# kubeflow/Code-Intelligence

Hardware: NVIDIA H100
Metric: issues/sec to 2400-d @ seq_len 512 batch 256 (higher is better)
Workload: dtype bf16

## Files before the change

code_intelligence_b200/csrc/api.cu:

```cuda
#include <algorithm>
#include <cmath>
#include <cstdarg>
#include <cstdio>
#include <cstdlib>
#include <cstring>
#include <mutex>
#include <string>
#include <vector>

#include <cuda_fp16.h>

#include "../../include/issue_emb_b200.h"
#include "kernels.h"

namespace {

thread_local std::string g_last_error;

int fail(int code, const char* fmt, ...) {
  char buf[512];
  va_list ap;
  va_start(ap, fmt);
  vsnprintf(buf, sizeof(buf), fmt, ap);
  va_end(ap);
// ... 375 lines not shown
    }
    if ((rc = mark(h, 1, s)) != IE_OK) return rc;
    int cur = 0;
    const __nv_bfloat16* layer_in = h->x0.as<__nv_bfloat16>();
    const __nv_bfloat16* prev_ring = nullptr;
    long long layer_in_ld = ring_mul * h->e_pad;
    for (int l = 0; l < c.n_layers; ++l) {
      const bool last = (l == c.n_layers - 1);
      Layer& L = h->layers[l];
      const bool from_table = proj && l == 0;
      const bool fused = persistent && last && l > 0 && h->segs == 1 && h->fuse_last && L.w_cat.p != nullptr;
      __nv_bfloat16* ybuf = h->y[cur].as<__nv_bfloat16>();
      __nv_bfloat16* carry = h->hcarry.as<__nv_bfloat16>() + static_cast<size_t>(l) * carry_layer;
      float* cstate = h->c.as<float>() + static_cast<size_t>(l) * h->max_batch * mop;
      CUtensorMap tm_h, tm_w;
      CK(ie::make_tmap_bf16_2d(&tm_h, ybuf, static_cast<uint64_t>(ring_mul) * L.kh_pad, static_cast<uint64_t>(crow + b_pad),
                               h->y_ld, 64, 128));
      if (fused)
        CK(ie::make_tmap_bf16_2d(&tm_w, L.w_cat.p, static_cast<uint64_t>(L.kin_pad + L.kh_pad), 4ull * L.out_pad,
                                 static_cast<uint64_t>(L.kin_pad + L.kh_pad), 64, 256));
      else
        CK(ie::make_tmap_bf16_2d(&tm_w, L.w_hh.p, static_cast<uint64_t>(ring_mul) * L.kh_pad, 4ull * L.out_pad,
                                 static_cast<uint64_t>(ring_mul) * L.kh_pad, 64, 256));
      CUtensorMap tm_h64 = tm_h;
      CUtensorMap tm_x = tm_h;
      if (fused)
        CK(ie::make_tmap_bf16_2d(&tm_x, prev_ring, static_cast<uint64_t>(L.kin_pad), static_cast<uint64_t>(crow + b_pad),
                                 h->y_ld, 64, 128));
      if (h->use_mc)
        CK(ie::make_tmap_bf16_2d(&tm_h64, ybuf, static_cast<uint64_t>(ring_mul) * L.kh_pad,
                                 static_cast<uint64_t>(crow + b_pad), h->y_ld, 64, 64));
      CK(cudaMemcpyAsync(ybuf, carry, slot_bytes, cudaMemcpyDeviceToDevice, s));
      if (!from_table && !fused) {
        ie::GemmArgs g{};
        fill_gemm(h, L, g);
        g.a = layer_in;
        g.lda = layer_in_ld;
        g.d = h->gx.p;
        g.m_pad = static_cast<int>(crow);
        g.m_store = static_cast<int>(crow);
        g.diag = h->diag.as<long long>() + 8 * l + 4;
        CK(ie::launch_gemm_bf16(g, s));
        h->launches++;
      }
      if ((rc = mark(h, 2 + 2 * l, s)) != IE_OK) return rc;

      if (persistent) CK(cudaMemsetAsync(h->step_done.p, 0, static_cast<size_t>(Tc) * ng * sizeof(unsigned), s));
      ie::LstmLayerArgs q{};
      q.tm_h = tm_h; q.tm_w = tm_w; q.tm_h64 = tm_h64; q.mc = h->use_mc; q.mc_ctas = h->mc_ctas;
      q.tm_x = tm_x; q.pre_nkb = fused ? L.kin_pad / 64 : 0; q.bias = L.bias.as<float>();
      q.gx = from_table ? h->proj.p : h->gx.p;
      q.tok = from_table ? h->tok.as<int>() : nullptr;
      q.c = cstate; q.y = ybuf;
      q.raw = (l == raw_layer && raw_out != nullptr) ? h->raw.as<float>() : nullptr;
      q.pool_sum = (last && pooled) ? h->pool_sum.as<float>() : nullptr;
      q.pool_max = h->pool_max.as<float>(); q.pool_last = h->pool_last.as<float>();
      q.lengths = h->lengths.as<int>();
      q.step_done = h->step_done.as<unsigned>();
      q.abort_flag = h->err.as<unsigned>() + 1; q.spin_limit = h->spin_limit;
      q.T = Tc; q.t0 = static_cast<int>(t0); q.T_total = T; q.ng = ng;
      q.u = L.u; q.n_cta = L.n_cta; q.out_pad = L.out_pad; q.kh_pad = L.kh_pad;
      q.ldy = h->y_ld; q.raw_ld = L.out_pad;
      q.gate_mode = h->gate_mode; q.gx_bf16 = h->gx_bf16; q.segs = h->segs;
      q.num_sms = h->num_sms; q.check_only = 0; q.cooperative = h->cooperative; q.fault = h->fault;
      q.diag = h->diag.as<long long>() + 8 * l;
// ... 844 lines not shown
```

code_intelligence_b200/csrc/gemm.cu:

```cuda
#include "gemm_kernel.cuh"

namespace ie {


cudaError_t launch_gemm_bf16(const GemmArgs& g, cudaStream_t stream) {
  if (g.m_pad % kBlockM || g.k_pad % kBlockK || g.bn % 16 || g.bn < 16 || g.bn > 256 || g.n_pad % g.bn ||
      g.n_store % 16 || g.ldd % 2)
    return cudaErrorInvalidValue;
  CUtensorMap tmA, tmB;
  const int segs = g.segs == 3 ? 3 : 1;
  const uint64_t k_inner = static_cast<uint64_t>(segs == 3 ? 2 : 1) * g.k_pad;
  const long long spin_limit = g.spin_limit > 0 ? g.spin_limit : kSpinLimitDefault;
  cudaError_t e = make_tmap_bf16_2d(&tmA, g.a, k_inner, g.m_pad, g.lda, kBlockK, kBlockM);
  if (e != cudaSuccess) return e;
  e = make_tmap_bf16_2d(&tmB, g.b, k_inner, g.n_pad, g.ldb, kBlockK, kBlockN);
  if (e != cudaSuccess) return e;

  const size_t smem = 1024 + static_cast<size_t>(kGemmStages) * kGemmStageBytes + 2 * kGemmStages * 8 + 32;
  const int num_m_blocks = g.m_pad / kBlockM;
  const int num_n_blocks = (g.n_pad + kBlockN - 1) / kBlockN;
  const int num_k_blocks = g.k_pad / kBlockK;
  const int num_tiles = num_m_blocks * num_n_blocks;
  const int sms = g.num_sms > 0 ? g.num_sms : 132;
  const int grid = num_tiles < sms ? num_tiles : sms;
  const int panel = 16;

#define IE_LAUNCH(OUT, ACT, FRAG)                                                                                  \
  do {                                                                                                             \
    auto kfn = gemm_bf16_kernel<OUT, ACT, FRAG>;                                                                       \
    e = cudaFuncSetAttribute(kfn, cudaFuncAttributeMaxDynamicSharedMemorySize, static_cast<int>(smem));            \
// ... 30 lines not shown
```

code_intelligence_b200/csrc/kernels.h:

```cpp
#pragma once
#include <cuda.h>
#include <cuda_bf16.h>
#include <cuda_runtime.h>
#include <stddef.h>
#include <stdint.h>

namespace ie {

cudaError_t make_tmap_bf16_2d(CUtensorMap* out, const void* base, uint64_t inner, uint64_t rows, uint64_t ld,
                              uint32_t box_inner, uint32_t box_rows);

__host__ __device__ inline int frag_index(int c, int elem_bytes) {
  const int q = (c & 7) >> 1;
  const int ix = 4 * (c >> 4) + 2 * ((c >> 3) & 1) + (c & 1);
  const int per_chunk = 16 / elem_bytes;
  return (ix / per_chunk * 4 + q) * per_chunk + ix % per_chunk;
}

struct GemmArgs {
  const __nv_bfloat16* a;
  const __nv_bfloat16* b;
  void* d;
  const float* bias;
  int m_pad, n_pad, k_pad;
  long long lda, ldb, ldd;
// ... 4 lines not shown
  int num_sms;
  int segs;
  unsigned* abort_flag;
  long long spin_limit;
  long long* diag;
  int frag;
};
cudaError_t launch_gemm_bf16(const GemmArgs& g, cudaStream_t stream);

constexpr int kMaxBatches = 12;
struct LstmLayerArgs {
  CUtensorMap tm_h;
  CUtensorMap tm_w;
  CUtensorMap tm_h64;
  CUtensorMap tm_x;
  int pre_nkb;
  const float* bias;
  int mc;
  int mc_ctas;
  const void* gx;
  const int* tok;
  float* c;
  __nv_bfloat16* y;
  float* raw;
  float* pool_sum;
  float* pool_max;
  float* pool_last;
  const int* lengths;
  unsigned* step_done;
  unsigned* abort_flag;
// ... 61 lines not shown
```

code_intelligence_b200/csrc/knn.cu:

```cuda
#include <algorithm>

#include "gemm_kernel.cuh"

namespace ie {

namespace {

__device__ __forceinline__ uint32_t order_key(float s) {
  const uint32_t b = __float_as_uint(s);
  return (b & 0x80000000u) ? ~b : (b | 0x80000000u);
}
__device__ __forceinline__ float key_score(uint32_t k) {
  return __uint_as_float((k & 0x80000000u) ? (k & 0x7fffffffu) : ~k);
}

__device__ __noinline__ float knn_compact(uint2* buf, int count, int kp, int lane) {
  __syncwarp();
  uint32_t t = 0;
  for (int bit = 31; bit >= 0; --bit) {
    const uint32_t c = t | (1u << bit);
    int m = 0;
    for (int i = lane; i < count; i += 32) m += buf[i].x >= c;
    if (static_cast<int>(__reduce_add_sync(~0u, static_cast<unsigned>(m))) >= kp) t = c;
  }
// ... 375 lines not shown
}

void knn_plan(int nq, long long n, int kp, int num_sms, int* S, int* nbs) {
  const int m_blocks = (nq + 127) / 128;
  const long long n_blocks = (n + 255) / 256;
  long long s = std::max(1, num_sms / m_blocks);
  s = std::min<long long>(s, n_blocks);
  s = std::min<long long>(s, kKnnMergeMax / kp);
  *nbs = static_cast<int>((n_blocks + s - 1) / s);
  *S = static_cast<int>((n_blocks + *nbs - 1) / *nbs);
}

cudaError_t launch_knn_stage1(const KnnStage1Args& a, cudaStream_t stream) {
  if (a.m_pad % 128 || a.k_pad % 64 || a.nq > a.m_pad) return cudaErrorInvalidValue;
  CUtensorMap tmA, tmB;
  cudaError_t e = make_tmap_bf16_2d(&tmA, a.qs, 2ull * a.k_pad, a.m_pad, 2ull * a.k_pad, kBlockK, kBlockM);
  if (e != cudaSuccess) return e;
  e = make_tmap_bf16_2d(&tmB, a.xs, 2ull * a.k_pad, static_cast<uint64_t>(a.n), 2ull * a.k_pad, kBlockK, kBlockN);
  if (e != cudaSuccess) return e;
  KnnEpi epi{};
  epi.cand = a.cand;
  epi.cnt = a.cnt;
  epi.col = a.col;
  epi.rowt = a.rowt;
  epi.nq = a.nq;
  epi.n = static_cast<int>(a.n);
  epi.S = a.S;
  epi.nbs = a.nbs;
  epi.kp = a.kp;
  epi.cosine = a.cosine;
  epi.m_blocks = a.m_pad / kBlockM;
  epi.items = epi.m_blocks * a.S;
  const int num_n_blocks = static_cast<int>((a.n + kBlockN - 1) / kBlockN);
// ... 25 lines not shown
```

code_intelligence_b200/csrc/lstm_common.cuh:

```cuda
#pragma once
#include <cuda_bf16.h>
#include <cuda_fp16.h>

#include "ptx.cuh"

namespace ie {

constexpr int kGatesFast = 2;
constexpr int kGatesExp = 1;
constexpr int kGatesIeee = 0;

__device__ __forceinline__ float sigmoid_ieee(float x) { return 1.0f / (1.0f + expf(-x)); }
__device__ __forceinline__ float tanh_ieee(float x) {
  const float ax = fabsf(x);
  float t;
  if (ax < 0.55f) {
    const float e = expm1f(2.0f * ax);
    t = e / (e + 2.0f);
  } else {
    t = 1.0f - 2.0f / (expf(2.0f * ax) + 1.0f);
  }
  return copysignf(t, x);
}

// ... 5 lines not shown
  } else if (gate_mode == kGatesExp) {
    cnew = sigmoid_acc(zf) * cprev + sigmoid_acc(zi) * tanh_acc(zg);
    hn = sigmoid_acc(zo) * tanh_acc(cnew);
  } else {
    cnew = sigmoid_ieee(zf) * cprev + sigmoid_ieee(zi) * tanh_ieee(zg);
    hn = sigmoid_ieee(zo) * tanh_ieee(cnew);
  }
}

__device__ __forceinline__ void red_add_v4_f32(float* p, float4 v) {
  asm volatile("red.relaxed.gpu.global.add.v4.f32 [%0], {%1, %2, %3, %4};" ::"l"(p), "f"(v.x), "f"(v.y), "f"(v.z),
               "f"(v.w)
               : "memory");
}
__device__ __forceinline__ void pool_accumulate4(float* pool_sum, float* pool_max, float* pool_last, long long po,
                                                 float4 hn, int tg, int len) {
  if (tg >= len) return;
  float4* mp = reinterpret_cast<float4*>(pool_max + po);
  if (tg == 0) {
    __stcg(reinterpret_cast<float4*>(pool_sum + po), hn);
    __stcg(mp, hn);
  } else {
    red_add_v4_f32(pool_sum + po, hn);
    const float4 m = __ldcg(mp);
    __stcg(mp, make_float4(fmaxf(m.x, hn.x), fmaxf(m.y, hn.y), fmaxf(m.z, hn.z), fmaxf(m.w, hn.w)));
  }
  if (tg == len - 1) __stcg(reinterpret_cast<float4*>(pool_last + po), hn);
}

__device__ __forceinline__ uint32_t enc_max(float x) {
  const uint32_t b = __float_as_uint(x);
  return (b & 0x80000000u) ? ~b : (b | 0x80000000u);
}
__host__ __device__ __forceinline__ float dec_max(uint32_t e) {
  const uint32_t b = (e & 0x80000000u) ? (e & 0x7FFFFFFFu) : ~e;
#ifdef __CUDA_ARCH__
  return __uint_as_float(b);
#else
  float f;
// ... 15 lines not shown
```

code_intelligence_b200/csrc/lstm_layer.cu:

```cuda
#include <cmath>

#include <cuda_fp16.h>

#include "kernels.h"
#include "lstm_common.cuh"
#include "ptx.cuh"

namespace ie {

namespace {

constexpr int kLThreads = 384;
constexpr int kLStages = 4;
constexpr int kLTileN = 256;
constexpr int kLRows = 128;
constexpr uint32_t kHBytes = kLRows * 64 * 2;
constexpr uint32_t kWBytes = kLTileN * 64 * 2;
constexpr uint32_t kStageBytes = kHBytes + kWBytes;

__device__ __forceinline__ void st_release_cta(uint32_t* p, uint32_t v) {
  asm volatile("st.release.cta.shared::cta.u32 [%0], %1;" ::"r"(smem_u32(p)), "r"(v) : "memory");
}
__device__ __forceinline__ uint32_t ld_acquire_cta(const uint32_t* p) {
  uint32_t v;
  asm volatile("ld.acquire.cta.shared::cta.u32 %0, [%1];" : "=r"(v) : "r"(smem_u32(p)) : "memory");
  return v;
}
__device__ __forceinline__ void wait_seq_ge(const uint32_t* p, uint32_t target, const Abort& ab) {
  if (ld_acquire_cta(p) >= target) return;
  if (aborted(ab)) return;
  const long long t0 = clock64();
  uint32_t spins = 0;
  while (ld_acquire_cta(p) < target) {
// ... 13 lines not shown
  float* pool_max;
  float* pool_last;
  const int* lengths;
  unsigned* step_done;
  unsigned* abort_flag;
  long long spin_limit;
  long long ldy, raw_ld;
  long long* trace;
  long long* diag;
  int T, t_begin, t0, T_total, ng, tiles, out_pad, nkb, segs, kh_pad, gate_mode, trace_items, fault;
  int pre_nkb;
};

template <bool TOK, bool GXBF, bool POOL, bool MC, bool FUSE>
__device__ __forceinline__ void lstm_layer_body(const CUtensorMap& tm_h, const CUtensorMap& tm_w,
                                                const CUtensorMap& tm_h64, const CUtensorMap& tm_x, const KArgs& a) {
  extern __shared__ uint8_t smem_raw[];
  const uint32_t rawaddr = smem_u32(smem_raw);
  uint8_t* smem = smem_raw + ((1024u - (rawaddr & 1023u)) & 1023u);

  uint8_t* ring = smem;
  uint64_t* full = reinterpret_cast<uint64_t*>(ring + kLStages * kStageBytes);
  uint64_t* empty = full + kLStages;
  uint32_t* cready = reinterpret_cast<uint32_t*>(empty + kLStages);
  uint32_t* abort_s = cready + 1;
  const Abort ab{abort_s, a.abort_flag, a.spin_limit};

  const int warp = threadIdx.x >> 5;
  const int lane = threadIdx.x & 31;
  long long* const trace = a.trace;
#define IE_TRACE(slot, kk) do { if (trace && (kk) < a.trace_items) { unsigned long long _g; \
    asm volatile("mov.u64 %0, %%globaltimer;" : "=l"(_g)); \
    trace[(static_cast<long long>(blockIdx.x) * a.trace_items + (kk)) * 12 + (slot)] = static_cast<long long>(_g); } } while (0)
  const uint32_t crank = MC ? cluster_ctarank() : 0u;
  const int P = static_cast<int>(gridDim.x);
  const int tiles = a.tiles, ng = a.ng;
  const int per_batch = 2 * tiles;
  const int C = ng * per_batch;
  const long long total = static_cast<long long>(a.T) * C;
  const int b_pad = 256 * ng;
// ... 2 lines not shown
  auto decode = [&](long long n, int& t, int& g, int& half, int& j) {
    const long long s = n / C;
    const int c = static_cast<int>(n - s * C);
    t = a.t_begin + static_cast<int>(s);
    g = c / per_batch;
    const int r = c - g * per_batch;
    half = r / tiles;
    j = r - half * tiles;
  };

  if (warp == 0 && lane == 0) {
    tma_prefetch_desc(&tm_h);
    tma_prefetch_desc(&tm_w);
    if (MC) tma_prefetch_desc(&tm_h64);
    if (FUSE) tma_prefetch_desc(&tm_x);
    if (a.diag != nullptr && blockIdx.x == 0) {
      unsigned long long g;
      asm volatile("mov.u64 %0, %%globaltimer;" : "=l"(g));
      a.diag[0] = clock64();
      a.diag[1] = static_cast<long long>(g);
    }
  }
  if (warp == 1 && lane == 0) {
    for (int s = 0; s < kLStages; ++s) {
      mbar_init(&full[s], 2);
      mbar_init(&empty[s], MC ? 4 : 2);
    }
    *cready = 0;
    *abort_s = 0;
    fence_barrier_init();
  }
  if (MC) cluster_sync();
  else __syncthreads();

  if (warp < 4) {
    if (warp == 0 && lane == 0) {
      int stage = 0;
      uint32_t phase = 0;
      int k = 0;
      for (long long n = blockIdx.x; n < total && !aborted(ab); n += P, ++k) {
        int t, g, half, j;
        decode(n, t, g, half, j);
        const int row0 = t * b_pad + g * 256 + half * kLRows;
        if constexpr (FUSE) {
// ... 8 lines not shown
        if (t > a.t_begin) fence_proxy_async();
        IE_TRACE(0, k);
        for (int kb = 0; kb < nkt; ++kb) {
          mbar_wait(&empty[stage], phase ^ 1, ab);
          mbar_arrive_expect_tx(&full[stage], kHBytes);
          const int seg = kb / a.nkb, r = kb - seg * a.nkb;
          const int kc = (seg == 1 ? a.kh_pad : 0) + r * 64;
          if constexpr (MC) {
            tma_load_2d_mc(ring + stage * kStageBytes + crank * (kHBytes / 2), &tm_h64, &full[stage], kc,
                           row0 + static_cast<int>(crank) * (kLRows / 2), static_cast<uint16_t>(0x3), kEvictNormal);
          } else {
            tma_load_2d(ring + stage * kStageBytes, &tm_h, &full[stage], kc, row0, kEvictNormal);
          }
          if (++stage == kLStages) { stage = 0; phase ^= 1; }
        }
        IE_TRACE(1, k);
      }
    } else if (warp == 1 && lane == 0) {
      int stage = 0;
      uint32_t phase = 0;
      for (long long n = blockIdx.x; n < total && !aborted(ab); n += P) {
        int t, g, half, j;
        decode(n, t, g, half, j);
        for (int kb = 0; kb < pre + nkt; ++kb) {
          mbar_wait(&empty[stage], phase ^ 1, ab);
          mbar_arrive_expect_tx(&full[stage], kWBytes);
          const int seg = FUSE ? 0 : kb / a.nkb, r = kb - seg * a.nkb;
          tma_load_2d(ring + stage * kStageBytes + kHBytes, &tm_w, &full[stage], (seg == 2 ? a.kh_pad : 0) + r * 64,
                      j * kLTileN, kEvictLast);
          if (++stage == kLStages) { stage = 0; phase ^= 1; }
        }
      }
    } else if (warp == 2 && lane == 0) {
      int k = 0;
      for (long long n = blockIdx.x; n < total && !aborted(ab); n += P, ++k) {
        int t, g, half, j;
        decode(n, t, g, half, j);
        if (t > a.t_begin)
          wait_flag_ge_relaxed(a.step_done + (t - a.t_begin - 1) * ng + g, static_cast<unsigned>(per_batch), ab);
        st_release_cta(cready, static_cast<uint32_t>(k + 1));
      }
    }
  } else {
    const int wg = (warp - 4) >> 2;
    const int q = lane & 3;
    const int rbase = wg * 64 + (warp & 3) * 16 + (lane >> 2);
    const long long lo_off = a.segs > 1 ? a.kh_pad : 0;
    const uint32_t ring_base = smem_u32(ring);
    const bool signal = (threadIdx.x & 127) == 0;
    int stage = 0;
    uint32_t phase = 0;
    int k = 0;
    float d[128];
    for (long long n = blockIdx.x; n < total; n += P, ++k) {
      int t, g, half, j;
// ... 15 lines not shown
          if (signal) {
            mbar_arrive(&empty[prev]);
            if (MC) mbar_arrive_remote(&empty[prev], crank ^ 1u);
          }
        }
        prev = stage;
        if (++stage == kLStages) { stage = 0; phase ^= 1; }
      }
      wgmma_wait<0>();
      wgmma_fence_regs(d);
      if (signal && prev >= 0) {
        mbar_arrive(&empty[prev]);
        if (MC) mbar_arrive_remote(&empty[prev], crank ^ 1u);
      }
      if (signal && wg == 0) IE_TRACE(3, k);
      if (lane == 0) wait_seq_ge(cready, static_cast<uint32_t>(k + 1), ab);
      __syncwarp();
#pragma unroll
      for (int hr = 0; hr < 2; ++hr) {
        const int brow = g * 256 + half * kLRows + rbase + 8 * hr;
        const int len = POOL ? a.lengths[brow] : 1;
        const long long grow = TOK ? static_cast<long long>(__ldg(a.tok + static_cast<long long>(tg) * b_pad + brow))
                                   : static_cast<long long>(t) * b_pad + brow;
        const int unit0 = j * 64 + 4 * q;
        float* cp = a.cstate + static_cast<long long>(brow) * a.out_pad + unit0;
        __nv_bfloat16* yrow = a.y + (static_cast<long long>(t + 1) * b_pad + brow) * a.ldy + unit0;
        const long long po = static_cast<long long>(brow) * a.out_pad + unit0;
        const long long gtile = grow * (4ll * a.out_pad) + j * kLTileN;
        const float* btile = FUSE ? a.bias + j * kLTileN : nullptr;
        if constexpr (FUSE) asm volatile("" : "+l"(btile));
#pragma unroll
        for (int s = 0; s < 4; ++s) {
          uint4 gh[2];
          if constexpr (GXBF && !FUSE) {
            const uint4* gp = reinterpret_cast<const uint4*>(reinterpret_cast<const __half*>(a.gx) + gtile) + q;
#pragma unroll
            for (int i = 0; i < 2; ++i) gh[i] = __ldcs(gp + 4 * (2 * s + i));
          }
          const float4 cprev = (tg == 0) ? make_float4(0.0f, 0.0f, 0.0f, 0.0f)
                                         : __ldcg(reinterpret_cast<const float4*>(cp + 16 * s));
          const float cp4[4] = {cprev.x, cprev.y, cprev.z, cprev.w};
          float cn[4], hn[4];
#pragma unroll
          for (int e = 0; e < 4; ++e) {
            const int m = 4 * s + e;
            float4 gx;
            if constexpr (FUSE) {
              gx = __ldg(reinterpret_cast<const float4*>(btile) + q + 4 * m);
            } else if constexpr (GXBF) {
              const uint32_t w0 = (e & 1) ? gh[e >> 1].z : gh[e >> 1].x, w1 = (e & 1) ? gh[e >> 1].w : gh[e >> 1].y;
              const float2 f01 = __half22float2(*reinterpret_cast<const __half2*>(&w0));
              const float2 f23 = __half22float2(*reinterpret_cast<const __half2*>(&w1));
              gx = make_float4(f01.x, f01.y, f23.x, f23.y);
            } else {
              gx = __ldcs(reinterpret_cast<const float4*>(reinterpret_cast<const float*>(a.gx) + gtile) + q + 4 * m);
            }
            const float zi = d[8 * m + 2 * hr] + gx.x;
            const float zf = d[8 * m + 2 * hr + 1] + gx.y;
            const float zg = d[8 * m + 4 + 2 * hr] + gx.z;
            const float zo = d[8 * m + 4 + 2 * hr + 1] + gx.w;
            lstm_cell1(zi, zf, zg, zo, cp4[e], cn[e], hn[e], a.gate_mode);
          }
          const float4 h4 = make_float4(hn[0], hn[1], hn[2], hn[3]);
          __stcg(reinterpret_cast<float4*>(cp + 16 * s), make_float4(cn[0], cn[1], cn[2], cn[3]));
          store_h4(yrow + 16 * s, h4, lo_off);
          if (a.raw != nullptr)
            *reinterpret_cast<float4*>(a.raw + (static_cast<long long>(brow) * a.T_total + tg) * a.raw_ld + unit0 + 16 * s) = h4;
          if constexpr (POOL) pool_accumulate4(a.pool_sum, a.pool_max, a.pool_last, po + 16 * s, h4, tg, len);
        }
      }
      named_bar_sync(1, 256);
      if (threadIdx.x == 128) {
        __threadfence();
        if (a.step_done != nullptr && !(a.fault && n == C))
          red_relaxed_add(a.step_done + (t - a.t_begin) * ng + g, 1u);
        IE_TRACE(6, k);
      }
    }
  }

  __syncwarp();
  if (MC) cluster_sync();
  if (a.diag != nullptr && threadIdx.x == 0 && blockIdx.x == 0) {
    unsigned long long g;
    asm volatile("mov.u64 %0, %%globaltimer;" : "=l"(g));
    a.diag[2] = clock64();
    a.diag[3] = static_cast<long long>(g);
  }
#undef IE_TRACE
}

thread_local int g_last_max_ctas = 0;

template <bool TOK, bool GXBF, bool POOL>
__global__ void __launch_bounds__(kLThreads, 1)
lstm_layer_kernel(const __grid_constant__ CUtensorMap tm_h, const __grid_constant__ CUtensorMap tm_w,
                  const __grid_constant__ CUtensorMap tm_h64, const __grid_constant__ CUtensorMap tm_x,
                  const __grid_constant__ KArgs a) {
  lstm_layer_body<TOK, GXBF, POOL, false, false>(tm_h, tm_w, tm_h64, tm_x, a);
}

template <bool POOL>
__global__ void __launch_bounds__(kLThreads, 1)
lstm_layer_fused_kernel(const __grid_constant__ CUtensorMap tm_h, const __grid_constant__ CUtensorMap tm_w,
                        const __grid_constant__ CUtensorMap tm_h64, const __grid_constant__ CUtensorMap tm_x,
                        const __grid_constant__ KArgs a) {
  lstm_layer_body<false, true, POOL, false, true>(tm_h, tm_w, tm_h64, tm_x, a);
}

template <bool TOK>
__global__ void __cluster_dims__(2, 1, 1) __launch_bounds__(kLThreads, 1)
lstm_layer_mc_kernel(const __grid_constant__ CUtensorMap tm_h, const __grid_constant__ CUtensorMap tm_w,
                     const __grid_constant__ CUtensorMap tm_h64, const __grid_constant__ CUtensorMap tm_x,
                     const __grid_constant__ KArgs a) {
  lstm_layer_body<TOK, true, false, true, false>(tm_h, tm_w, tm_h64, tm_x, a);
}

size_t layer_smem_bytes() { return 1024 + static_cast<size_t>(kLStages) * kStageBytes + 2 * kLStages * 8 + 32; }

template <bool TOK, bool GXBF, bool POOL, bool MC, bool FUSE = false>
cudaError_t launch_layer_t(const LstmLayerArgs& a, int ctas, int tiles, cudaStream_t stream) {
  void (*kfn)(CUtensorMap, CUtensorMap, CUtensorMap, CUtensorMap, KArgs);
  if constexpr (MC) kfn = lstm_layer_mc_kernel<TOK>;
  else if constexpr (FUSE) kfn = lstm_layer_fused_kernel<POOL>;
  else kfn = lstm_layer_kernel<TOK, GXBF, POOL>;
  const size_t smem = layer_smem_bytes();
  cudaError_t e = cudaFuncSetAttribute(kfn, cudaFuncAttributeMaxDynamicSharedMemorySize, static_cast<int>(smem));
  if (e != cudaSuccess) return e;
  if (a.check_only) {
    int max_ctas = 0;
    if (MC) {
      cudaLaunchConfig_t cfg{};
      cfg.gridDim = dim3(2 * (a.num_sms / 2));
      cfg.blockDim = dim3(kLThreads);
      cfg.dynamicSmemBytes = smem;
      cfg.stream = stream;
      int clusters = 0;
// ... 21 lines not shown
  k.trace_items = a.trace_items; k.fault = a.fault;
  cudaLaunchConfig_t cfg{};
  cfg.gridDim = dim3(ctas);
  cfg.blockDim = dim3(kLThreads);
  cfg.dynamicSmemBytes = smem;
  cfg.stream = stream;
  cudaLaunchAttribute attr[1];
  int na = 0;
  if (a.cooperative && !a.single_step) {
    attr[na].id = cudaLaunchAttributeCooperative;
    attr[na].val.cooperative = 1;
    ++na;
  }
  cfg.attrs = attr;
  cfg.numAttrs = na;
  return cudaLaunchKernelEx(&cfg, kfn, a.tm_h, a.tm_w, a.tm_h64, FUSE ? a.tm_x : a.tm_h, k);
}

bool lstm_layer_mc_ok(const LstmLayerArgs& a) {
  return a.mc != 0 && !a.single_step && a.gx_bf16 && a.pool_sum == nullptr && a.pre_nkb == 0 && a.segs == 1 &&
         (a.n_cta / 2) % 2 == 0 && a.mc_ctas >= 2;
}

}

int lstm_layer_max_ctas() { return g_last_max_ctas; }

int lstm_layer_ctas(const LstmLayerArgs& a) {
  const long long per_step = static_cast<long long>(a.ng) * a.n_cta;
  if (a.single_step) return static_cast<int>(per_step);
  const long long total = a.T * per_step;
// ... 32 lines not shown
```

code_intelligence_b200/csrc/misc.cu:

```cuda
#include <cstring>

#include "kernels.h"
#include "lstm_common.cuh"
#include "ptx.cuh"

namespace ie {

typedef CUresult (*EncodeTiledFn)(CUtensorMap*, CUtensorMapDataType, cuuint32_t, void*, const cuuint64_t*,
                                  const cuuint64_t*, const cuuint32_t*, const cuuint32_t*, CUtensorMapInterleave,
                                  CUtensorMapSwizzle, CUtensorMapL2promotion, CUtensorMapFloatOOBfill);

static EncodeTiledFn get_encode_fn() {
  static EncodeTiledFn fn = nullptr;
  if (fn == nullptr) {
    void* p = nullptr;
    cudaDriverEntryPointQueryResult q;
    if (cudaGetDriverEntryPoint("cuTensorMapEncodeTiled", &p, cudaEnableDefault, &q) == cudaSuccess &&
        q == cudaDriverEntryPointSuccess)
      fn = reinterpret_cast<EncodeTiledFn>(p);
  }
  return fn;
}

cudaError_t make_tmap_bf16_2d(CUtensorMap* out, const void* base, uint64_t inner, uint64_t rows, uint64_t ld,
                              uint32_t box_inner, uint32_t box_rows) {
  EncodeTiledFn fn = get_encode_fn();
  if (fn == nullptr) return cudaErrorNotSupported;
  if (box_inner != 64 || box_rows == 0 || box_rows > 256 || (ld * 2) % 16 != 0 ||
      (reinterpret_cast<uintptr_t>(base) & 15) != 0)
    return cudaErrorInvalidValue;
  cuuint64_t dims[2] = {inner, rows};
  cuuint64_t strides[1] = {ld * 2};
  cuuint32_t box[2] = {box_inner, box_rows};
  cuuint32_t estr[2] = {1, 1};
  CUresult r = fn(out, CU_TENSOR_MAP_DATA_TYPE_BFLOAT16, 2, const_cast<void*>(base), dims, strides, box, estr,
                  CU_TENSOR_MAP_INTERLEAVE_NONE, CU_TENSOR_MAP_SWIZZLE_128B, CU_TENSOR_MAP_L2_PROMOTION_L2_256B,
                  CU_TENSOR_MAP_FLOAT_OOB_FILL_NONE);
  return r == CUDA_SUCCESS ? cudaSuccess : cudaErrorInvalidValue;
}

namespace {

__global__ void embed_gather_kernel(const int64_t* __restrict__ ids, int B, int T, int b_pad,
                                    const uint4* __restrict__ emb, int vocab, int chunks ,
                                    uint4* __restrict__ x0, long long ldx_chunks, int pad_idx, int* err_flag, int t0, int Tc) {
  const int warps_per_block = blockDim.x >> 5;
  const long long row = static_cast<long long>(blockIdx.x) * warps_per_block + (threadIdx.x >> 5);
  const long long total = static_cast<long long>(Tc) * b_pad;
  if (row >= total) return;
  const int lane = threadIdx.x & 31;
  const int tl = static_cast<int>(row / b_pad);
  const int b = static_cast<int>(row - static_cast<long long>(tl) * b_pad);
// ... 157 lines not shown
```

code_intelligence_b200/csrc/ptx.cuh:

```cuda
#pragma once
#include <cuda.h>
#include <cuda_bf16.h>
#include <cuda_runtime.h>
#include <stdint.h>

namespace ie {

constexpr uint64_t kEvictNormal = 0x1000000000000000ull;
constexpr uint64_t kEvictFirst  = 0x12F0000000000000ull;
constexpr uint64_t kEvictLast   = 0x14F0000000000000ull;

__device__ __forceinline__ uint32_t smem_u32(const void* p) {
  return static_cast<uint32_t>(__cvta_generic_to_shared(p));
}

__device__ __forceinline__ void mbar_init(uint64_t* bar, uint32_t count) {
  asm volatile("mbarrier.init.shared::cta.b64 [%0], %1;" ::"r"(smem_u32(bar)), "r"(count) : "memory");
}
__device__ __forceinline__ void fence_barrier_init() {
  asm volatile("fence.mbarrier_init.release.cluster;" ::: "memory");
}
__device__ __forceinline__ void fence_proxy_async() { asm volatile("fence.proxy.async;" ::: "memory"); }

__device__ __forceinline__ void mbar_arrive(uint64_t* bar) {
// ... 62 lines not shown
  while (!mbar_try_wait(bar, parity)) {
    if (((++spins) & 0xFFu) == 0 && abort_poll(ab, t0)) return;
  }
}

__device__ __forceinline__ void tma_prefetch_desc(const CUtensorMap* m) {
  asm volatile("prefetch.tensormap [%0];" ::"l"(m) : "memory");
}
__device__ __forceinline__ void tma_load_2d(void* smem_dst, const CUtensorMap* m, uint64_t* bar, int32_t c0,
                                            int32_t c1, uint64_t hint) {
  asm volatile(
      "cp.async.bulk.tensor.2d.shared::cluster.global.mbarrier::complete_tx::bytes.L2::cache_hint"
      " [%0], [%1, {%3, %4}], [%2], %5;"
      ::"r"(smem_u32(smem_dst)), "l"(m), "r"(smem_u32(bar)), "r"(c0), "r"(c1), "l"(hint)
      : "memory");
}

__device__ __forceinline__ void tma_load_2d_mc(void* smem_dst, const CUtensorMap* m, uint64_t* bar, int32_t c0,
                                               int32_t c1, uint16_t mask, uint64_t hint) {
  asm volatile(
      "cp.async.bulk.tensor.2d.shared::cluster.global.mbarrier::complete_tx::bytes.multicast::cluster.L2::cache_hint"
      " [%0], [%1, {%4, %5}], [%2], %3, %6;"
      ::"r"(smem_u32(smem_dst)), "l"(m), "r"(smem_u32(bar)), "h"(mask), "r"(c0), "r"(c1), "l"(hint)
      : "memory");
}

__device__ __forceinline__ uint32_t cluster_ctarank() {
  uint32_t r;
  asm volatile("mov.u32 %0, %%cluster_ctarank;" : "=r"(r));
  return r;
// ... 98 lines not shown
```

Baseline: 3896.

## Prefetch LSTM epilogue gate inputs and cell state into smem via TMA

The epilogue of the persistent LSTM layer kernel used to read precomputed gate inputs (gx), the previous cell state and the running pool max straight from global memory. Those reads now become TMA and bulk-copy loads issued by the producer warps into extra pipeline stages, so they overlap with the recurrent GEMM mainloop. The token-table path gets a dedicated warp that prefetches gathered rows to L2 and bulk-loads them. This adds two ring stages per tile, a more involved stage and phase bookkeeping between producers and consumers, and a generalized tensor-map helper, which raises the risk of pipeline hazards.

```diff
diff --git a/code_intelligence_b200/csrc/api.cu b/code_intelligence_b200/csrc/api.cu
--- a/code_intelligence_b200/csrc/api.cu
+++ b/code_intelligence_b200/csrc/api.cu
@@ -413,22 +413,33 @@
       __nv_bfloat16* carry = h->hcarry.as<__nv_bfloat16>() + static_cast<size_t>(l) * carry_layer;
       float* cstate = h->c.as<float>() + static_cast<size_t>(l) * h->max_batch * mop;
       CUtensorMap tm_h, tm_w;
-      CK(ie::make_tmap_bf16_2d(&tm_h, ybuf, static_cast<uint64_t>(ring_mul) * L.kh_pad, static_cast<uint64_t>(crow + b_pad),
-                               h->y_ld, 64, 128));
+      CK(ie::make_tmap_2d(&tm_h, ybuf, static_cast<uint64_t>(ring_mul) * L.kh_pad, static_cast<uint64_t>(crow + b_pad),
+                          h->y_ld, 64, 128));
       if (fused)
-        CK(ie::make_tmap_bf16_2d(&tm_w, L.w_cat.p, static_cast<uint64_t>(L.kin_pad + L.kh_pad), 4ull * L.out_pad,
-                                 static_cast<uint64_t>(L.kin_pad + L.kh_pad), 64, 256));
+        CK(ie::make_tmap_2d(&tm_w, L.w_cat.p, static_cast<uint64_t>(L.kin_pad + L.kh_pad), 4ull * L.out_pad,
+                            static_cast<uint64_t>(L.kin_pad + L.kh_pad), 64, 256));
       else
-        CK(ie::make_tmap_bf16_2d(&tm_w, L.w_hh.p, static_cast<uint64_t>(ring_mul) * L.kh_pad, 4ull * L.out_pad,
-                                 static_cast<uint64_t>(ring_mul) * L.kh_pad, 64, 256));
+        CK(ie::make_tmap_2d(&tm_w, L.w_hh.p, static_cast<uint64_t>(ring_mul) * L.kh_pad, 4ull * L.out_pad,
+                            static_cast<uint64_t>(ring_mul) * L.kh_pad, 64, 256));
       CUtensorMap tm_h64 = tm_h;
       CUtensorMap tm_x = tm_h;
       if (fused)
-        CK(ie::make_tmap_bf16_2d(&tm_x, prev_ring, static_cast<uint64_t>(L.kin_pad), static_cast<uint64_t>(crow + b_pad),
-                                 h->y_ld, 64, 128));
+        CK(ie::make_tmap_2d(&tm_x, prev_ring, static_cast<uint64_t>(L.kin_pad), static_cast<uint64_t>(crow + b_pad),
+                            h->y_ld, 64, 128));
       if (h->use_mc)
-        CK(ie::make_tmap_bf16_2d(&tm_h64, ybuf, static_cast<uint64_t>(ring_mul) * L.kh_pad,
-                                 static_cast<uint64_t>(crow + b_pad), h->y_ld, 64, 64));
+        CK(ie::make_tmap_2d(&tm_h64, ybuf, static_cast<uint64_t>(ring_mul) * L.kh_pad,
+                            static_cast<uint64_t>(crow + b_pad), h->y_ld, 64, 64));
+      CUtensorMap tm_gx = tm_h, tm_c, tm_pmax = tm_h;
+      if (!from_table && !fused && h->gx_bf16)
+        CK(ie::make_tmap_2d(&tm_gx, h->gx.p, 4ull * L.out_pad, static_cast<uint64_t>(crow), 4ull * L.out_pad, 256, 64,
+                            CU_TENSOR_MAP_DATA_TYPE_FLOAT16, CU_TENSOR_MAP_SWIZZLE_NONE));
+      CK(ie::make_tmap_2d(&tm_c, cstate, static_cast<uint64_t>(L.out_pad), static_cast<uint64_t>(b_pad),
+                          static_cast<uint64_t>(L.out_pad), 64, 64, CU_TENSOR_MAP_DATA_TYPE_FLOAT32,
+                          CU_TENSOR_MAP_SWIZZLE_NONE));
+      if (fused && pooled)
+        CK(ie::make_tmap_2d(&tm_pmax, h->pool_max.p, static_cast<uint64_t>(L.out_pad), static_cast<uint64_t>(b_pad),
+                            static_cast<uint64_t>(L.out_pad), 64, 64, CU_TENSOR_MAP_DATA_TYPE_FLOAT32,
+                            CU_TENSOR_MAP_SWIZZLE_NONE));
       CK(cudaMemcpyAsync(ybuf, carry, slot_bytes, cudaMemcpyDeviceToDevice, s));
       if (!from_table && !fused) {
         ie::GemmArgs g{};
@@ -448,6 +459,7 @@
       ie::LstmLayerArgs q{};
       q.tm_h = tm_h; q.tm_w = tm_w; q.tm_h64 = tm_h64; q.mc = h->use_mc; q.mc_ctas = h->mc_ctas;
       q.tm_x = tm_x; q.pre_nkb = fused ? L.kin_pad / 64 : 0; q.bias = L.bias.as<float>();
+      q.tm_gx = tm_gx; q.tm_c = tm_c; q.tm_pmax = tm_pmax;
       q.gx = from_table ? h->proj.p : h->gx.p;
       q.tok = from_table ? h->tok.as<int>() : nullptr;
       q.c = cstate; q.y = ybuf;
diff --git a/code_intelligence_b200/csrc/gemm.cu b/code_intelligence_b200/csrc/gemm.cu
--- a/code_intelligence_b200/csrc/gemm.cu
+++ b/code_intelligence_b200/csrc/gemm.cu
@@ -11,9 +11,9 @@
   const int segs = g.segs == 3 ? 3 : 1;
   const uint64_t k_inner = static_cast<uint64_t>(segs == 3 ? 2 : 1) * g.k_pad;
   const long long spin_limit = g.spin_limit > 0 ? g.spin_limit : kSpinLimitDefault;
-  cudaError_t e = make_tmap_bf16_2d(&tmA, g.a, k_inner, g.m_pad, g.lda, kBlockK, kBlockM);
+  cudaError_t e = make_tmap_2d(&tmA, g.a, k_inner, g.m_pad, g.lda, kBlockK, kBlockM);
   if (e != cudaSuccess) return e;
-  e = make_tmap_bf16_2d(&tmB, g.b, k_inner, g.n_pad, g.ldb, kBlockK, kBlockN);
+  e = make_tmap_2d(&tmB, g.b, k_inner, g.n_pad, g.ldb, kBlockK, kBlockN);
   if (e != cudaSuccess) return e;
 
   const size_t smem = 1024 + static_cast<size_t>(kGemmStages) * kGemmStageBytes + 2 * kGemmStages * 8 + 32;
diff --git a/code_intelligence_b200/csrc/kernels.h b/code_intelligence_b200/csrc/kernels.h
--- a/code_intelligence_b200/csrc/kernels.h
+++ b/code_intelligence_b200/csrc/kernels.h
@@ -7,8 +7,10 @@
 
 namespace ie {
 
-cudaError_t make_tmap_bf16_2d(CUtensorMap* out, const void* base, uint64_t inner, uint64_t rows, uint64_t ld,
-                              uint32_t box_inner, uint32_t box_rows);
+cudaError_t make_tmap_2d(CUtensorMap* out, const void* base, uint64_t inner, uint64_t rows, uint64_t ld,
+                         uint32_t box_inner, uint32_t box_rows,
+                         CUtensorMapDataType dtype = CU_TENSOR_MAP_DATA_TYPE_BFLOAT16,
+                         CUtensorMapSwizzle swizzle = CU_TENSOR_MAP_SWIZZLE_128B);
 
 __host__ __device__ inline int frag_index(int c, int elem_bytes) {
   const int q = (c & 7) >> 1;
@@ -43,6 +45,9 @@
   CUtensorMap tm_w;
   CUtensorMap tm_h64;
   CUtensorMap tm_x;
+  CUtensorMap tm_gx;
+  CUtensorMap tm_c;
+  CUtensorMap tm_pmax;
   int pre_nkb;
   const float* bias;
   int mc;
diff --git a/code_intelligence_b200/csrc/knn.cu b/code_intelligence_b200/csrc/knn.cu
--- a/code_intelligence_b200/csrc/knn.cu
+++ b/code_intelligence_b200/csrc/knn.cu
@@ -413,9 +413,9 @@
 cudaError_t launch_knn_stage1(const KnnStage1Args& a, cudaStream_t stream) {
   if (a.m_pad % 128 || a.k_pad % 64 || a.nq > a.m_pad) return cudaErrorInvalidValue;
   CUtensorMap tmA, tmB;
-  cudaError_t e = make_tmap_bf16_2d(&tmA, a.qs, 2ull * a.k_pad, a.m_pad, 2ull * a.k_pad, kBlockK, kBlockM);
+  cudaError_t e = make_tmap_2d(&tmA, a.qs, 2ull * a.k_pad, a.m_pad, 2ull * a.k_pad, kBlockK, kBlockM);
   if (e != cudaSuccess) return e;
-  e = make_tmap_bf16_2d(&tmB, a.xs, 2ull * a.k_pad, static_cast<uint64_t>(a.n), 2ull * a.k_pad, kBlockK, kBlockN);
+  e = make_tmap_2d(&tmB, a.xs, 2ull * a.k_pad, static_cast<uint64_t>(a.n), 2ull * a.k_pad, kBlockK, kBlockN);
   if (e != cudaSuccess) return e;
   KnnEpi epi{};
   epi.cand = a.cand;
diff --git a/code_intelligence_b200/csrc/lstm_common.cuh b/code_intelligence_b200/csrc/lstm_common.cuh
--- a/code_intelligence_b200/csrc/lstm_common.cuh
+++ b/code_intelligence_b200/csrc/lstm_common.cuh
@@ -43,7 +43,7 @@
                : "memory");
 }
 __device__ __forceinline__ void pool_accumulate4(float* pool_sum, float* pool_max, float* pool_last, long long po,
-                                                 float4 hn, int tg, int len) {
+                                                 float4 hn, int tg, int len, const float* max_sm) {
   if (tg >= len) return;
   float4* mp = reinterpret_cast<float4*>(pool_max + po);
   if (tg == 0) {
@@ -51,7 +51,7 @@
     __stcg(mp, hn);
   } else {
     red_add_v4_f32(pool_sum + po, hn);
-    const float4 m = __ldcg(mp);
+    const float4 m = max_sm != nullptr ? *reinterpret_cast<const float4*>(max_sm) : __ldcg(mp);
     __stcg(mp, make_float4(fmaxf(m.x, hn.x), fmaxf(m.y, hn.y), fmaxf(m.z, hn.z), fmaxf(m.w, hn.w)));
   }
   if (tg == len - 1) __stcg(reinterpret_cast<float4*>(pool_last + po), hn);
diff --git a/code_intelligence_b200/csrc/lstm_layer.cu b/code_intelligence_b200/csrc/lstm_layer.cu
--- a/code_intelligence_b200/csrc/lstm_layer.cu
+++ b/code_intelligence_b200/csrc/lstm_layer.cu
@@ -17,6 +17,9 @@
 constexpr uint32_t kHBytes = kLRows * 64 * 2;
 constexpr uint32_t kWBytes = kLTileN * 64 * 2;
 constexpr uint32_t kStageBytes = kHBytes + kWBytes;
+constexpr uint32_t kEpiGxBytes = 64 * kLTileN * 2;
+constexpr uint32_t kEpiCBytes = 64 * 64 * 4;
+static_assert(kEpiGxBytes + kEpiCBytes <= kStageBytes && 2 * kEpiCBytes <= kStageBytes, "entry exceeds a stage");
 
 __device__ __forceinline__ void st_release_cta(uint32_t* p, uint32_t v) {
   asm volatile("st.release.cta.shared::cta.u32 [%0], %1;" ::"r"(smem_u32(p)), "r"(v) : "memory");
@@ -60,7 +63,13 @@
 
 template <bool TOK, bool GXBF, bool POOL, bool MC, bool FUSE>
 __device__ __forceinline__ void lstm_layer_body(const CUtensorMap& tm_h, const CUtensorMap& tm_w,
-                                                const CUtensorMap& tm_h64, const CUtensorMap& tm_x, const KArgs& a) {
+                                                const CUtensorMap& tm_h64, const CUtensorMap& tm_x,
+                                                const CUtensorMap& tm_gx, const CUtensorMap& tm_c,
+                                                const CUtensorMap& tm_pmax, const KArgs& a) {
+  constexpr bool kGxSm = GXBF && !FUSE;
+  constexpr bool kMaxSm = POOL && FUSE;
+  constexpr uint32_t kCOff = kGxSm ? kEpiGxBytes : 0u;
+  constexpr uint32_t kCBytes = kMaxSm ? 2 * kEpiCBytes : kEpiCBytes;
   extern __shared__ uint8_t smem_raw[];
   const uint32_t rawaddr = smem_u32(smem_raw);
   uint8_t* smem = smem_raw + ((1024u - (rawaddr & 1023u)) & 1023u);
@@ -70,6 +79,7 @@
   uint64_t* empty = full + kLStages;
   uint32_t* cready = reinterpret_cast<uint32_t*>(empty + kLStages);
   uint32_t* abort_s = cready + 1;
+  uint32_t* gready = cready + 2;
   const Abort ab{abort_s, a.abort_flag, a.spin_limit};
 
   const int warp = threadIdx.x >> 5;
@@ -102,6 +112,9 @@
     tma_prefetch_desc(&tm_w);
     if (MC) tma_prefetch_desc(&tm_h64);
     if (FUSE) tma_prefetch_desc(&tm_x);
+    if (kGxSm && !TOK) tma_prefetch_desc(&tm_gx);
+    tma_prefetch_desc(&tm_c);
+    if (kMaxSm) tma_prefetch_desc(&tm_pmax);
     if (a.diag != nullptr && blockIdx.x == 0) {
       unsigned long long g;
       asm volatile("mov.u64 %0, %%globaltimer;" : "=l"(g));
@@ -116,6 +129,7 @@
     }
     *cready = 0;
     *abort_s = 0;
+    *gready = 0;
     fence_barrier_init();
   }
   if (MC) cluster_sync();
@@ -154,12 +168,22 @@
           }
           if (++stage == kLStages) { stage = 0; phase ^= 1; }
         }
+        for (int e = 0; e < 2; ++e) {
+          mbar_wait(&empty[stage], phase ^ 1, ab);
+          mbar_arrive_expect_tx(&full[stage], kCBytes);
+          uint8_t* dst = ring + stage * kStageBytes + kCOff;
+          const int brow0 = g * 256 + half * kLRows + e * 64;
+          tma_load_2d(dst, &tm_c, &full[stage], j * 64, brow0, kEvictNormal);
+          if constexpr (kMaxSm) tma_load_2d(dst + kEpiCBytes, &tm_pmax, &full[stage], j * 64, brow0, kEvictNormal);
+          if (++stage == kLStages) { stage = 0; phase ^= 1; }
+        }
         IE_TRACE(1, k);
       }
     } else if (warp == 1 && lane == 0) {
       int stage = 0;
       uint32_t phase = 0;
-      for (long long n = blockIdx.x; n < total && !aborted(ab); n += P) {
+      int kw = 0;
+      for (long long n = blockIdx.x; n < total && !aborted(ab); n += P, ++kw) {
         int t, g, half, j;
         decode(n, t, g, half, j);
         for (int kb = 0; kb < pre + nkt; ++kb) {
@@ -170,6 +194,20 @@
                       j * kLTileN, kEvictLast);
           if (++stage == kLStages) { stage = 0; phase ^= 1; }
         }
+        for (int e = 0; e < 2; ++e) {
+          mbar_wait(&empty[stage], phase ^ 1, ab);
+          if constexpr (!kGxSm) {
+            mbar_arrive(&full[stage]);
+          } else if constexpr (TOK) {
+            st_release_cta(gready, static_cast<uint32_t>(2 * kw + e + 1));
+          } else {
+            mbar_arrive_expect_tx(&full[stage], kEpiGxBytes);
+            uint8_t* dst = ring + stage * kStageBytes;
+            const int brow0 = g * 256 + half * kLRows + e * 64;
+            tma_load_2d(dst, &tm_gx, &full[stage], j * kLTileN, t * b_pad + brow0, kEvictFirst);
+          }
+          if (++stage == kLStages) { stage = 0; phase ^= 1; }
+        }
       }
     } else if (warp == 2 && lane == 0) {
       int k = 0;
@@ -179,6 +217,37 @@
         if (t > a.t_begin)
           wait_flag_ge_relaxed(a.step_done + (t - a.t_begin - 1) * ng + g, static_cast<unsigned>(per_batch), ab);
         st_release_cta(cready, static_cast<uint32_t>(k + 1));
+      }
+    } else if (warp == 3) {
+      if constexpr (kGxSm && TOK) {
+        int stage = 0;
+        uint32_t phase = 0;
+        int kg = 0;
+        for (long long n = blockIdx.x; n < total && !aborted(ab); n += P, ++kg) {
+          int t, g, half, j;
+          decode(n, t, g, half, j);
+          const int* tp = a.tok + static_cast<long long>(a.t0 + t) * b_pad + g * 256 + half * kLRows + lane;
+          int id[4];
+#pragma unroll
+          for (int i = 0; i < 4; ++i) id[i] = __ldg(tp + 32 * i);
+          const __half* tab = reinterpret_cast<const __half*>(a.gx) + j * kLTileN;
+          const long long pitch = 4ll * a.out_pad;
+#pragma unroll
+          for (int i = 0; i < 4; ++i) bulk_prefetch_l2(tab + id[i] * pitch, kLTileN * 2);
+          for (int kb = 0; kb < pre + nkt; ++kb)
+            if (++stage == kLStages) { stage = 0; phase ^= 1; }
+#pragma unroll
+          for (int e = 0; e < 2; ++e) {
+            wait_seq_ge(gready, static_cast<uint32_t>(2 * kg + e + 1), ab);
+            if (lane == 0) mbar_arrive_expect_tx(&full[stage], kEpiGxBytes);
+            uint8_t* dst = ring + stage * kStageBytes;
+#pragma unroll
+            for (int i = 0; i < 2; ++i)
+              bulk_load_1d(dst + (32 * i + lane) * (kLTileN * 2), tab + id[2 * e + i] * pitch, kLTileN * 2, &full[stage],
+                           kEvictFirst);
+            if (++stage == kLStages) { stage = 0; phase ^= 1; }
+          }
+        }
       }
     }
   } else {
@@ -224,31 +293,44 @@
         if (MC) mbar_arrive_remote(&empty[prev], crank ^ 1u);
       }
       if (signal && wg == 0) IE_TRACE(3, k);
-      if (lane == 0) wait_seq_ge(cready, static_cast<uint32_t>(k + 1), ab);
-      __syncwarp();
+      if (wg == 1 && ++stage == kLStages) { stage = 0; phase ^= 1; }
+      mbar_wait(&full[stage], phase, ab);
+      if (signal && wg == 0) IE_TRACE(4, k);
+      const uint8_t* ent = ring + stage * kStageBytes;
+      if (++stage == kLStages) { stage = 0; phase ^= 1; }
+      if (wg == 0 && ++stage == kLStages) { stage = 0; phase ^= 1; }
+      if constexpr (POOL && !FUSE) {
+        if (lane == 0) wait_seq_ge(cready, static_cast<uint32_t>(k + 1), ab);
+        __syncwarp();
+      }
 #pragma unroll
       for (int hr = 0; hr < 2; ++hr) {
         const int brow = g * 256 + half * kLRows + rbase + 8 * hr;
+        const int rl = rbase - wg * 64 + 8 * hr;
         const int len = POOL ? a.lengths[brow] : 1;
-        const long long grow = TOK ? static_cast<long long>(__ldg(a.tok + static_cast<long long>(tg) * b_pad + brow))
-                                   : static_cast<long long>(t) * b_pad + brow;
         const int unit0 = j * 64 + 4 * q;
         float* cp = a.cstate + static_cast<long long>(brow) * a.out_pad + unit0;
         __nv_bfloat16* yrow = a.y + (static_cast<long long>(t + 1) * b_pad + brow) * a.ldy + unit0;
         const long long po = static_cast<long long>(brow) * a.out_pad + unit0;
-        const long long gtile = grow * (4ll * a.out_pad) + j * kLTileN;
+        const float* cs = reinterpret_cast<const float*>(ent + kCOff + rl * 256) + 4 * q;
+        const uint4* gs = reinterpret_cast<const uint4*>(ent + rl * (kLTileN * 2)) + q;
+        long long gtile = 0;
+        if constexpr (!kGxSm && !FUSE) {
+          const long long grow = TOK ? static_cast<long long>(__ldg(a.tok + static_cast<long long>(tg) * b_pad + brow))
+                                     : static_cast<long long>(t) * b_pad + brow;
+          gtile = grow * (4ll * a.out_pad) + j * kLTileN;
+        }
         const float* btile = FUSE ? a.bias + j * kLTileN : nullptr;
         if constexpr (FUSE) asm volatile("" : "+l"(btile));
 #pragma unroll
         for (int s = 0; s < 4; ++s) {
           uint4 gh[2];
-          if constexpr (GXBF && !FUSE) {
-            const uint4* gp = reinterpret_cast<const uint4*>(reinterpret_cast<const __half*>(a.gx) + gtile) + q;
-#pragma unroll
-            for (int i = 0; i < 2; ++i) gh[i] = __ldcs(gp + 4 * (2 * s + i));
+          if constexpr (kGxSm) {
+#pragma unroll
+            for (int i = 0; i < 2; ++i) gh[i] = gs[4 * (2 * s + i)];
           }
           const float4 cprev = (tg == 0) ? make_float4(0.0f, 0.0f, 0.0f, 0.0f)
-                                         : __ldcg(reinterpret_cast<const float4*>(cp + 16 * s));
+                                         : *reinterpret_cast<const float4*>(cs + 16 * s);
           const float cp4[4] = {cprev.x, cprev.y, cprev.z, cprev.w};
           float cn[4], hn[4];
 #pragma unroll
@@ -272,14 +354,24 @@
             lstm_cell1(zi, zf, zg, zo, cp4[e], cn[e], hn[e], a.gate_mode);
           }
           const float4 h4 = make_float4(hn[0], hn[1], hn[2], hn[3]);
-          __stcg(reinterpret_cast<float4*>(cp + 16 * s), make_float4(cn[0], cn[1], cn[2], cn[3]));
+          __stcg(reinterpret_cast<float4*>((POOL ? a.cstate + po : cp) + 16 * s), make_float4(cn[0], cn[1], cn[2], cn[3]));
           store_h4(yrow + 16 * s, h4, lo_off);
           if (a.raw != nullptr)
             *reinterpret_cast<float4*>(a.raw + (static_cast<long long>(brow) * a.T_total + tg) * a.raw_ld + unit0 + 16 * s) = h4;
-          if constexpr (POOL) pool_accumulate4(a.pool_sum, a.pool_max, a.pool_last, po + 16 * s, h4, tg, len);
+          if constexpr (POOL)
+            pool_accumulate4(a.pool_sum, a.pool_max, a.pool_last, po + 16 * s, h4, tg, len,
+                             kMaxSm ? cs + kEpiCBytes / 4 + 16 * s : nullptr);
         }
       }
       named_bar_sync(1, 256);
+      if (signal) {
+#pragma unroll
+        for (int e = 1; e <= 2; ++e) {
+          const int es = (stage + kLStages - e) % kLStages;
+          mbar_arrive(&empty[es]);
+          if (MC) mbar_arrive_remote(&empty[es], crank ^ 1u);
+        }
+      }
       if (threadIdx.x == 128) {
         __threadfence();
         if (a.step_done != nullptr && !(a.fault && n == C))
@@ -306,31 +398,34 @@
 __global__ void __launch_bounds__(kLThreads, 1)
 lstm_layer_kernel(const __grid_constant__ CUtensorMap tm_h, const __grid_constant__ CUtensorMap tm_w,
                   const __grid_constant__ CUtensorMap tm_h64, const __grid_constant__ CUtensorMap tm_x,
-                  const __grid_constant__ KArgs a) {
-  lstm_layer_body<TOK, GXBF, POOL, false, false>(tm_h, tm_w, tm_h64, tm_x, a);
+                  const __grid_constant__ CUtensorMap tm_gx, const __grid_constant__ CUtensorMap tm_c,
+                  const __grid_constant__ CUtensorMap tm_pmax, const __grid_constant__ KArgs a) {
+  lstm_layer_body<TOK, GXBF, POOL, false, false>(tm_h, tm_w, tm_h64, tm_x, tm_gx, tm_c, tm_pmax, a);
 }
 
 template <bool POOL>
 __global__ void __launch_bounds__(kLThreads, 1)
 lstm_layer_fused_kernel(const __grid_constant__ CUtensorMap tm_h, const __grid_constant__ CUtensorMap tm_w,
                         const __grid_constant__ CUtensorMap tm_h64, const __grid_constant__ CUtensorMap tm_x,
-                        const __grid_constant__ KArgs a) {
-  lstm_layer_body<false, true, POOL, false, true>(tm_h, tm_w, tm_h64, tm_x, a);
+                        const __grid_constant__ CUtensorMap tm_gx, const __grid_constant__ CUtensorMap tm_c,
+                        const __grid_constant__ CUtensorMap tm_pmax, const __grid_constant__ KArgs a) {
+  lstm_layer_body<false, true, POOL, false, true>(tm_h, tm_w, tm_h64, tm_x, tm_gx, tm_c, tm_pmax, a);
 }
 
 template <bool TOK>
 __global__ void __cluster_dims__(2, 1, 1) __launch_bounds__(kLThreads, 1)
 lstm_layer_mc_kernel(const __grid_constant__ CUtensorMap tm_h, const __grid_constant__ CUtensorMap tm_w,
                      const __grid_constant__ CUtensorMap tm_h64, const __grid_constant__ CUtensorMap tm_x,
-                     const __grid_constant__ KArgs a) {
-  lstm_layer_body<TOK, true, false, true, false>(tm_h, tm_w, tm_h64, tm_x, a);
+                     const __grid_constant__ CUtensorMap tm_gx, const __grid_constant__ CUtensorMap tm_c,
+                     const __grid_constant__ CUtensorMap tm_pmax, const __grid_constant__ KArgs a) {
+  lstm_layer_body<TOK, true, false, true, false>(tm_h, tm_w, tm_h64, tm_x, tm_gx, tm_c, tm_pmax, a);
 }
 
 size_t layer_smem_bytes() { return 1024 + static_cast<size_t>(kLStages) * kStageBytes + 2 * kLStages * 8 + 32; }
 
 template <bool TOK, bool GXBF, bool POOL, bool MC, bool FUSE = false>
 cudaError_t launch_layer_t(const LstmLayerArgs& a, int ctas, int tiles, cudaStream_t stream) {
-  void (*kfn)(CUtensorMap, CUtensorMap, CUtensorMap, CUtensorMap, KArgs);
+  void (*kfn)(CUtensorMap, CUtensorMap, CUtensorMap, CUtensorMap, CUtensorMap, CUtensorMap, CUtensorMap, KArgs);
   if constexpr (MC) kfn = lstm_layer_mc_kernel<TOK>;
   else if constexpr (FUSE) kfn = lstm_layer_fused_kernel<POOL>;
   else kfn = lstm_layer_kernel<TOK, GXBF, POOL>;
@@ -382,7 +477,8 @@
   }
   cfg.attrs = attr;
   cfg.numAttrs = na;
-  return cudaLaunchKernelEx(&cfg, kfn, a.tm_h, a.tm_w, a.tm_h64, FUSE ? a.tm_x : a.tm_h, k);
+  return cudaLaunchKernelEx(&cfg, kfn, a.tm_h, a.tm_w, a.tm_h64, FUSE ? a.tm_x : a.tm_h,
+                            (GXBF && !FUSE && !TOK) ? a.tm_gx : a.tm_h, a.tm_c, (FUSE && POOL) ? a.tm_pmax : a.tm_h, k);
 }
 
 bool lstm_layer_mc_ok(const LstmLayerArgs& a) {
diff --git a/code_intelligence_b200/csrc/misc.cu b/code_intelligence_b200/csrc/misc.cu
--- a/code_intelligence_b200/csrc/misc.cu
+++ b/code_intelligence_b200/csrc/misc.cu
@@ -22,20 +22,25 @@
   return fn;
 }
 
-cudaError_t make_tmap_bf16_2d(CUtensorMap* out, const void* base, uint64_t inner, uint64_t rows, uint64_t ld,
-                              uint32_t box_inner, uint32_t box_rows) {
+cudaError_t make_tmap_2d(CUtensorMap* out, const void* base, uint64_t inner, uint64_t rows, uint64_t ld,
+                         uint32_t box_inner, uint32_t box_rows, CUtensorMapDataType dtype, CUtensorMapSwizzle swizzle) {
   EncodeTiledFn fn = get_encode_fn();
   if (fn == nullptr) return cudaErrorNotSupported;
-  if (box_inner != 64 || box_rows == 0 || box_rows > 256 || (ld * 2) % 16 != 0 ||
+  uint32_t esz = 0;
+  if (dtype == CU_TENSOR_MAP_DATA_TYPE_BFLOAT16 || dtype == CU_TENSOR_MAP_DATA_TYPE_FLOAT16) esz = 2;
+  if (dtype == CU_TENSOR_MAP_DATA_TYPE_FLOAT32) esz = 4;
+  const bool box_ok = swizzle == CU_TENSOR_MAP_SWIZZLE_128B ? box_inner * esz == 128
+                    : swizzle == CU_TENSOR_MAP_SWIZZLE_NONE ? box_inner <= 256 && (box_inner * esz) % 16 == 0
+                                                            : false;
+  if (esz == 0 || box_inner == 0 || !box_ok || box_rows == 0 || box_rows > 256 || (ld * esz) % 16 != 0 ||
       (reinterpret_cast<uintptr_t>(base) & 15) != 0)
     return cudaErrorInvalidValue;
   cuuint64_t dims[2] = {inner, rows};
-  cuuint64_t strides[1] = {ld * 2};
+  cuuint64_t strides[1] = {ld * esz};
   cuuint32_t box[2] = {box_inner, box_rows};
   cuuint32_t estr[2] = {1, 1};
-  CUresult r = fn(out, CU_TENSOR_MAP_DATA_TYPE_BFLOAT16, 2, const_cast<void*>(base), dims, strides, box, estr,
-                  CU_TENSOR_MAP_INTERLEAVE_NONE, CU_TENSOR_MAP_SWIZZLE_128B, CU_TENSOR_MAP_L2_PROMOTION_L2_256B,
-                  CU_TENSOR_MAP_FLOAT_OOB_FILL_NONE);
+  CUresult r = fn(out, dtype, 2, const_cast<void*>(base), dims, strides, box, estr, CU_TENSOR_MAP_INTERLEAVE_NONE,
+                  swizzle, CU_TENSOR_MAP_L2_PROMOTION_L2_256B, CU_TENSOR_MAP_FLOAT_OOB_FILL_NONE);
   return r == CUDA_SUCCESS ? cudaSuccess : cudaErrorInvalidValue;
 }
 
diff --git a/code_intelligence_b200/csrc/ptx.cuh b/code_intelligence_b200/csrc/ptx.cuh
--- a/code_intelligence_b200/csrc/ptx.cuh
+++ b/code_intelligence_b200/csrc/ptx.cuh
@@ -100,6 +100,18 @@
       " [%0], [%1, {%3, %4}], [%2], %5;"
       ::"r"(smem_u32(smem_dst)), "l"(m), "r"(smem_u32(bar)), "r"(c0), "r"(c1), "l"(hint)
       : "memory");
+}
+
+__device__ __forceinline__ void bulk_load_1d(void* smem_dst, const void* src, uint32_t bytes, uint64_t* bar,
+                                             uint64_t hint) {
+  asm volatile(
+      "cp.async.bulk.shared::cluster.global.mbarrier::complete_tx::bytes.L2::cache_hint [%0], [%1], %2, [%3], %4;"
+      ::"r"(smem_u32(smem_dst)), "l"(src), "r"(bytes), "r"(smem_u32(bar)), "l"(hint)
+      : "memory");
+}
+
+__device__ __forceinline__ void bulk_prefetch_l2(const void* src, uint32_t bytes) {
+  asm volatile("cp.async.bulk.prefetch.L2.global [%0], %1;" ::"l"(src), "r"(bytes) : "memory");
 }
 
 __device__ __forceinline__ void tma_load_2d_mc(void* smem_dst, const CUtensorMap* m, uint64_t* bar, int32_t c0,
```

After: 3909, median of 6. No clear change (+0.3%).
